# AnthonyDickson/HIVE

Hardware: AMD Instinct MI355X
Metric: frames/sec (depth+TSDF integrate) @640x480, 512^3 vol (higher is better)
Workload: dtype bf16; 1 GPU; synthetic 640x480x150 RGB (seeded room trajectory), host-resident uint8 frames uploaded in the timed region, DPT-Hybrid depth (seeded random weights: depth 1-7 m, bf16, hip engine) + 512x512x512 TSDF integrate, 107 frames/step; frames_total=4066, volume=512x512x512, tsdf_overlap=True, scaling_mode=weak

## Files before the change

### hive_amd/csrc/capi.hip

```cpp
#include <algorithm>

#include "hive_internal.hpp"

static thread_local std::string g_global_error;

void hive_set_global_error(const char *msg) { g_global_error = msg ? msg : ""; }

int hive_fail(hive_ctx *ctx, int code, const char *fmt, ...) {
    char buf[1024];
    va_list ap;
    va_start(ap, fmt);
    vsnprintf(buf, sizeof(buf), fmt, ap);
    va_end(ap);
    if (ctx)
        ctx->last_error = buf;
    else
        g_global_error = buf;
    return code;
}

int hive_reserve_device(hive_ctx *ctx, void **ptr, size_t *cur, size_t bytes) {
    if (*cur >= bytes && *ptr) return HIVE_OK;
    if (*ptr) {
        HIVE_CHECK_HIP(ctx, hipStreamSynchronize(ctx->stream));
// ... 103 lines not shown
            e = hipDeviceGetStreamPriorityRange(&least, &greatest);
            if (e == hipSuccess) e = hipStreamCreateWithPriority(&ctx->stream, hipStreamNonBlocking, least);
            ctx->owns_stream = true;
        } else {
            ctx->stream = (hipStream_t)stream;
        }
    }
    if (e == hipSuccess) e = hipMalloc((void **)&ctx->d_scalars, 4096 * sizeof(unsigned));
    if (e == hipSuccess) e = hipMemset(ctx->d_scalars, 0, 4096 * sizeof(unsigned));
    if (e == hipSuccess) e = hipMalloc(&ctx->d_zeros, 256);
    if (e == hipSuccess) e = hipMemset(ctx->d_zeros, 0, 256);
    if (e != hipSuccess) {
        int rc = hive_fail(nullptr, HIVE_ERR_DEVICE, "hive_ctx_create: %s", hipGetErrorString(e));
        delete ctx;
        return rc;
    }
    *out = ctx;
    return HIVE_OK;
}

int hive_ctx_destroy(hive_ctx *ctx) {
    if (!ctx) return HIVE_OK;
    {
        HIVE_ENTER(ctx);
        (void)hipStreamSynchronize(ctx->stream);
    for (auto &s : ctx->slots) {
        if (s.pinned) (void)hipHostFree(s.pinned);
        if (s.done) (void)hipEventDestroy(s.done);
    }
    for (auto ev : ctx->ev_pool) (void)hipEventDestroy(ev);
    if (ctx->d_scratch) (void)hipFree(ctx->d_scratch);
    if (ctx->d_frame) (void)hipFree(ctx->d_frame);
    if (ctx->d_batch) (void)hipFree(ctx->d_batch);
    if (ctx->d_gram) (void)hipFree(ctx->d_gram);
    if (ctx->d_splitk) (void)hipFree(ctx->d_splitk);
    if (ctx->d_splitk_count) (void)hipFree(ctx->d_splitk_count);
    if (ctx->d_in) (void)hipFree(ctx->d_in);
    if (ctx->d_scalars) (void)hipFree(ctx->d_scalars);
    if (ctx->h_pinned_small) (void)hipHostFree(ctx->h_pinned_small);
        if (ctx->d_zeros) (void)hipFree(ctx->d_zeros);
        if (ctx->owns_stream) (void)hipStreamDestroy(ctx->stream);
    }
    delete ctx;
    return HIVE_OK;
}

int hive_ctx_release_stream(hive_ctx *ctx) {
    if (!ctx) return hive_fail(nullptr, HIVE_ERR_INVALID, "ctx is NULL");
    ctx->owns_stream = false;
    return HIVE_OK;
}

int hive_ctx_set_stream(hive_ctx *ctx, void *stream) {
    HIVE_ENTER(ctx);
    if (!ctx) return hive_fail(nullptr, HIVE_ERR_INVALID, "ctx is NULL");
    HIVE_REQUIRE(ctx, stream != HIVE_STREAM_OWN && stream != HIVE_STREAM_OWN_LOW, "hive_ctx_set_stream: pass a hipStream_t (NULL = the default stream)");
    hipStream_t next = (hipStream_t)stream;
    if (next == ctx->stream) return HIVE_OK;
    hipEvent_t ev;
    HIVE_CHECK_HIP(ctx, hipEventCreateWithFlags(&ev, hipEventDisableTiming));
    hipError_t e = hipEventRecord(ev, ctx->stream);
    if (e == hipSuccess) e = hipStreamWaitEvent(next, ev, 0);
    (void)hipEventDestroy(ev);
    HIVE_CHECK_HIP(ctx, e);
    if (ctx->owns_stream) {
        (void)hipStreamSynchronize(ctx->stream);
// ... 82 lines not shown
```

### hive_amd/csrc/hive_internal.hpp

```cpp
#pragma once
#include <hip/hip_runtime.h>

#include <cstdarg>
#include <cstdint>
#include <cstdio>
#include <cstring>
#include <string>
#include <vector>

#include "../../include/hive_mi355x.h"

#define HIVE_WAVE 64

struct hive_staging_slot {
    void *pinned = nullptr;
    size_t bytes = 0;
    hipEvent_t done = nullptr;
    bool in_flight = false;
};

struct hive_ctx {
    int device = 0;
    int num_cus = 256;
    hipStream_t stream = nullptr;
    bool owns_stream = false;
    int round_mode = HIVE_ROUND_HALF_EVEN;
    std::string last_error;

    static constexpr int kSlots = 4;
    hive_staging_slot slots[kSlots];
    int next_slot = 0;

    void *d_scratch = nullptr;
    size_t scratch_bytes = 0;
    void *d_frame = nullptr;
    size_t frame_bytes = 0;
    void *d_batch = nullptr;
    size_t batch_bytes = 0;
    void *d_in = nullptr;
    size_t in_bytes = 0;
    int tsdf_scalars = 0;
    int tsdf_multi_scalars = 0;
    unsigned *d_scalars = nullptr;
    void *h_pinned_small = nullptr;
    void *d_zeros = nullptr;
    void *d_splitk = nullptr;
    size_t splitk_bytes = 0;
    unsigned *d_splitk_count = nullptr;
    void *d_gram = nullptr;
    size_t gram_bytes = 0;

    bool deterministic = false;
    int64_t n_splitk_launches = 0, n_deep_ring_launches = 0;

    bool timing = false;
    std::vector<hipEvent_t> ev_pool;
    size_t ev_used = 0;
    hipEvent_t last_start = nullptr, last_stop = nullptr;
};

int hive_fail(hive_ctx *ctx, int code, const char *fmt, ...);

struct hive_device_guard {
    int prev = -1;
    bool switched = false;
    explicit hive_device_guard(const hive_ctx *ctx) {
        if (!ctx) return;
        if (hipGetDevice(&prev) == hipSuccess && prev != ctx->device) switched = hipSetDevice(ctx->device) == hipSuccess;
    }
    ~hive_device_guard() {
        if (switched) (void)hipSetDevice(prev);
    }
    hive_device_guard(const hive_device_guard &) = delete;
    hive_device_guard &operator=(const hive_device_guard &) = delete;
};
// ... 93 lines not shown
```

### hive_amd/csrc/tsdf.hip

```cpp
#include "hive_internal.hpp"

#include <algorithm>
#include <cmath>
#include <cstdlib>
#include <type_traits>

struct FrameParams {
    float R[9];
    float T[3];
    float fx, fy, cx, cy;
    float ox, oy, oz, vs, trunc, obs_w;
    int X, Y, Z, H, W;
    int x_off;
    const uint2 *frame;
    const unsigned *tile_max;
    int tile_shift, tiles_x, tiles_y;
    int row_far;
    int fast_colour;
    unsigned long long *n_updated;
};

template <bool VEC>
__global__ __launch_bounds__(256) void prep_frame_kernel(const float *__restrict__ depth, const uint8_t *__restrict__ color, int H, int W, int tile_shift,
                                                         int tiles_x, uint2 *__restrict__ out, unsigned *__restrict__ tile_max, int tile_stride,
// ... 564 lines not shown
                vol_store4(v2 + idx, c, nrow);
            } else {
                vol_store4(v0 + plane + idx, w, nrow);
                vol_store4(v0 + 2 * plane + idx, c, nrow);
                vol_store4(v0 + 3 * plane + idx, c3, nrow);
                vol_store4(v0 + 4 * plane + idx, c4, nrow);
            }
        }
    }
    if (COUNT) {
        __shared__ unsigned wave_cnt[4];
        for (int off = 32; off > 0; off >>= 1) n_upd += __shfl_xor((int)n_upd, off);
        if (lane == 0) wave_cnt[threadIdx.x >> 6] = n_upd;
        __syncthreads();
        if (threadIdx.x == 0) {
            const unsigned total = wave_cnt[0] + wave_cnt[1] + wave_cnt[2] + wave_cnt[3];
            if (total) atomicAdd(p.n_updated + (size_t)(blockIdx.x % COUNT_SLOTS) * COUNT_STRIDE, (unsigned long long)total);
        }
    }
}

#ifndef HIVE_TSDF_MAXF
#define HIVE_TSDF_MAXF 4
#endif
constexpr int MAXF = HIVE_TSDF_MAXF;
static_assert(MAXF <= 4, "WorkItem::zz holds a 4-bit frame mask");
struct MultiParams {
    FrameParams f[MAXF];
    int nf;
    int frame_skip;
    int xcd_split;
    int bins_x;
    unsigned *clear_next;
    int lanes_along_x;
    int quad_interleave;
};

constexpr int MS_BASE = 2304, MS_STRIDE = 512, MS_NITEMS = MAXF, MS_HIST = 8, MS_CURSOR = MS_HIST + NBINS, MS_CLEAR = MS_CURSOR + NBINS;

__global__ __launch_bounds__(1024) void build_worklist_multi_kernel(MultiParams mp, WorkItem *__restrict__ items, unsigned *n_items, unsigned *hist) {
    __shared__ unsigned wave_sum[16];
    __shared__ unsigned block_base;
    __shared__ float dil[MAXF][MAX_TILES];
    __shared__ unsigned gmax[MAXF];
    __shared__ float gsum[MAXF];
    __shared__ unsigned bin_count[NBINS];
    constexpr int CHUNK = SEG_LANES * VPT;
    const FrameParams &p = mp.f[0];
    if (threadIdx.x < MAXF) gmax[threadIdx.x] = 0u, gsum[threadIdx.x] = 0.f;
    if (threadIdx.x < NBINS) bin_count[threadIdx.x] = 0u;
    __syncthreads();
    for (int f = 0; f < mp.nf; ++f) load_dilated_tiles(mp.f[f].tile_max, p.tiles_x, p.tiles_y, dil[f], &gmax[f], &gsum[f], threadIdx.x, 1024);
    __syncthreads();
    const long long row = (long long)blockIdx.x * 1024 + threadIdx.x;
    unsigned n_chunks = 0;
    int zstart = 0, z1 = 0, x = 0, y = 0;
    int fz0[MAXF], fz1[MAXF];
    float ax0 = 0.f, ay0 = 0.f, az0 = 0.f;
    auto frames_of = [&](int zs) {
        unsigned mask = 0;
#pragma unroll
        for (int f = 0; f < MAXF; ++f) mask |= (fz1[f] > zs && fz0[f] < zs + CHUNK) ? (1u << f) : 0u;
        return mask;
    };
    if (row < (long long)p.X * p.Y) {
        if (mp.lanes_along_x) {
            y = (int)(row / p.X);
            x = (int)(row % p.X);
        } else {
            x = (int)(row / p.Y);
            y = (int)(row % p.Y);
        }
        int lo = p.Z, hi = 0;
#pragma unroll
        for (int f = 0; f < MAXF; ++f) {
            fz0[f] = fz1[f] = 0;
            if (f < mp.nf) {
                const FrameParams &q = mp.f[f];
                const float tx = (q.ox + (float)(x + q.x_off) * q.vs) - q.T[0];
                const float ty = (q.oy + (float)y * q.vs) - q.T[1];
                const float ax = q.R[0] * tx + q.R[3] * ty;
                const float ay = q.R[1] * tx + q.R[4] * ty;
                const float az = q.R[2] * tx + q.R[5] * ty;
                if (f == 0) ax0 = ax, ay0 = ay, az0 = az;
                const bool row_far = p.row_far == 2 || (p.row_far == 1 && row_far_pays(gsum[f], gmax[f], p.tiles_x * p.tiles_y));
                const RowClip clip = clip_row(q, ax, ay, az, __uint_as_float(gmax[f]), row_far ? dil[f] : nullptr);
                if (clip.z1 > clip.z0) {
                    fz0[f] = clip.z0, fz1[f] = clip.z1;
                    lo = min(lo, clip.z0);
                    hi = max(hi, clip.z1);
                }
            }
        }
        if (hi > lo) {
            zstart = (lo / VPT) * VPT;
            z1 = hi;
            for (int zs = zstart; zs < z1; zs += CHUNK) n_chunks += frames_of(zs) ? 1u : 0u;
        }
    }
    const unsigned first = worklist_slots(n_chunks, n_items, wave_sum, &block_base);
    const int lane = threadIdx.x & 63;
    const unsigned quad_first = (unsigned)__shfl((int)first, lane & ~3);
    unsigned nq[4];
#pragma unroll
    for (int j = 0; j < 4; ++j) nq[j] = (unsigned)__shfl((int)n_chunks, (lane & ~3) + j);
    unsigned e = 0;
    if (n_chunks)
        for (int zs = zstart; zs < z1; zs += CHUNK) {
            const unsigned mask = frames_of(zs);
            if (!mask) continue;
            unsigned slot = quad_first;
            if (mp.quad_interleave) {
#pragma unroll
                for (int j = 0; j < 4; ++j) slot += min(nq[j], e) + ((j < (lane & 3) && nq[j] > e) ? 1u : 0u);
            } else {
                slot = first + e;
            }
            ++e;
            const float tz = (p.oz + (float)(zs + CHUNK / 2) * p.vs) - p.T[2];
            const float cz = az0 + p.R[8] * tz;
            const float v = cz > 1.0e-6f ? p.fy * ((ay0 + p.R[7] * tz) / cz) + p.cy : 0.f;
            const int bins_y = NBINS / mp.bins_x;
            int bin = min(max((int)(v * ((float)bins_y / (float)p.H)), 0), bins_y - 1);
            if (mp.bins_x > 1) {
                const float u = cz > 1.0e-6f ? p.fx * ((ax0 + p.R[6] * tz) / cz) + p.cx : 0.f;
                bin = bin * mp.bins_x + min(max((int)(u * ((float)mp.bins_x / (float)p.W)), 0), mp.bins_x - 1);
            }
            atomicAdd(&bin_count[bin], 1u);
            WorkItem it;
            it.xy = (unsigned)x | ((unsigned)y << 16);
            it.zz = (unsigned)zs | ((unsigned)(min(z1 - zs, CHUNK) - 1) << ITEM_NLIVE_SHIFT) | (mask << ITEM_MASK_SHIFT) | ((unsigned)bin << ITEM_BIN_SHIFT);
            items[slot] = it;
        }
    __syncthreads();
    if (threadIdx.x < NBINS && bin_count[threadIdx.x]) atomicAdd(hist + threadIdx.x, bin_count[threadIdx.x]);
}

__global__ __launch_bounds__(1024) void sort_worklist_kernel(const WorkItem *__restrict__ tmp, WorkItem *__restrict__ out, const unsigned *__restrict__ n_items_ptr,
                                                             const unsigned *__restrict__ hist, unsigned *cursor) {
    __shared__ unsigned base[NBINS], cnt[NBINS], gofs[NBINS];
    const unsigned n = *n_items_ptr;
    const unsigned i0 = blockIdx.x * 1024u;
    if (i0 >= n) return;
    if (threadIdx.x < NBINS) cnt[threadIdx.x] = 0u;
    if (threadIdx.x == 0) {
        unsigned a = 0;
        for (int b = 0; b < NBINS; ++b) {
            base[b] = a;
            a += hist[b];
        }
    }
    __syncthreads();
    const unsigned i = i0 + threadIdx.x;
    const int lane = threadIdx.x & 63;
    WorkItem it;
    it.xy = it.zz = 0u;
    unsigned bin = 0xffffffffu;
    if (i < n) {
        it = tmp[i];
        bin = it.zz >> ITEM_BIN_SHIFT;
    }
    unsigned rank = 0, wave_base = 0;
    unsigned long long todo = __ballot(i < n);
    while (todo) {
        const int leader = __ffsll((long long)todo) - 1;
        const unsigned b = (unsigned)__shfl((int)bin, leader);
        const unsigned long long m = __ballot(bin == b);
        unsigned wb = 0;
        if (lane == leader) wb = atomicAdd(&cnt[b], (unsigned)__popcll(m));
        wb = (unsigned)__shfl((int)wb, leader);
        if (bin == b) {
            rank = (unsigned)__popcll(m & ((1ull << lane) - 1ull));
            wave_base = wb;
        }
        todo &= ~m;
    }
    __syncthreads();
    if (threadIdx.x < NBINS && cnt[threadIdx.x]) gofs[threadIdx.x] = atomicAdd(cursor + threadIdx.x, cnt[threadIdx.x]);
    __syncthreads();
    if (i < n) out[base[bin] + gofs[bin] + wave_base + rank] = it;
}

#ifdef HIVE_TSDF_WAVES
#define HIVE_TSDF_OCC __attribute__((amdgpu_waves_per_eu(HIVE_TSDF_WAVES, HIVE_TSDF_WAVES)))
#else
#define HIVE_TSDF_OCC
#endif
template <int RM, int UPD>
__global__ __launch_bounds__(256) HIVE_TSDF_OCC void integrate_multi_kernel(MultiParams mp, const WorkItem *__restrict__ items, const unsigned *__restrict__ n_items_ptr,
                                                              float *__restrict__ v0, float *__restrict__ v1, float *__restrict__ v2) {
    constexpr int PER_WAVE = 64 / SEG_LANES, SEG_VOX = SEG_LANES * 4;
    typedef ItemShape Sh;
    typedef Sh::V V;
    __shared__ uint2 xchg[4 * PER_WAVE * SEG_VOX];
    const int lane = threadIdx.x & 63;
    const int seg = lane / SEG_LANES, sl = lane % SEG_LANES;
    const unsigned n_items = *n_items_ptr;
    const unsigned n_trips = (n_items + PER_WAVE - 1) / PER_WAVE;
    const unsigned per_xcd = mp.xcd_split ? (n_trips + 7u) / 8u : n_trips;
    const unsigned xcd = mp.xcd_split ? (blockIdx.x & 7u) : 0u;
    const unsigned local_block = mp.xcd_split ? (blockIdx.x >> 3) : blockIdx.x;
    const unsigned stride = (mp.xcd_split ? (gridDim.x >> 3) : gridDim.x) * 4;
    const unsigned trip_end = min(n_trips, (xcd + 1u) * per_xcd);
    const FrameParams &p0 = mp.f[0];
    const float trunc_rcp = refined_rcp(p0.trunc);
    if (blockIdx.x == 0 && (int)threadIdx.x < MS_CLEAR) mp.clear_next[threadIdx.x] = 0u;
    for (unsigned trip = xcd * per_xcd + local_block * 4 + (threadIdx.x >> 6); trip < trip_end; trip += stride) {
        const unsigned ii = trip * PER_WAVE + (unsigned)seg;
        WorkItem item;
        item.xy = item.zz = 0u;
        if (ii < n_items) item = items[ii];
        const int x = (int)(item.xy & 0xffffu), y = (int)(item.xy >> 16);
        const int zseg = (int)(item.zz & 0xffffu);
        const int zb = zseg + sl * VPT;
        const bool live = sl * VPT < item_nlive(item.zz);
        const int nrow = p0.Z - zb;
        const long long idx = ((long long)x * p0.Y + y) * p0.Z + zb;
        unsigned wave_frames = (item.zz >> ITEM_MASK_SHIFT) & 15u;
#pragma unroll
        for (int o = SEG_LANES; o < 64; o <<= 1) wave_frames |= (unsigned)__shfl_xor((int)wave_frames, o);
        wave_frames = mp.frame_skip ? (unsigned)__builtin_amdgcn_readfirstlane((int)wave_frames) : 0xffu;
        float t[VPT], w[VPT], cr[VPT], cg[VPT], cb[VPT];
        bool loaded = false;
        uint2 *mine = xchg + ((threadIdx.x >> 6) * PER_WAVE + seg) * SEG_VOX;
#pragma unroll 1
        for (int f = 0; f < mp.nf; ++f) {
            if (!((wave_frames >> f) & 1u)) continue;
            const FrameParams &p = mp.f[f];
            const float tx = (p.ox + (float)(x + p.x_off) * p.vs) - p.T[0];
            const float ty = (p.oy + (float)y * p.vs) - p.T[1];
            const float ax = p.R[0] * tx + p.R[3] * ty;
            const float ay = p.R[1] * tx + p.R[4] * ty;
            const float az = p.R[2] * tx + p.R[5] * ty;
            uint2 tex[4];
#pragma unroll
            for (int g = 0; g < 2; ++g) {
                V cz;
                int pix[Sh::NV];
                voxel_pixels<RM, V, Sh::NV, SEG_LANES>(p, ax, ay, az, zseg + sl + 2 * SEG_LANES * g, cz, pix);
// ... 216 lines not shown
    p.fy = K[4];
    p.cx = K[2];
    p.cy = K[5];
    p.ox = v->origin[0];
    p.oy = v->origin[1];
    p.oz = v->origin[2];
    p.vs = v->voxel_size;
    p.trunc = v->trunc;
    p.obs_w = obs_weight;
    p.X = (int)v->dim[0];
    p.x_off = (int)v->x_off;
    p.Y = (int)v->dim[1];
    p.Z = (int)v->dim[2];
    p.H = H;
    p.W = W;
    const TileGrid tg = tile_grid(H, W);
    p.tile_shift = tg.shift;
    p.tiles_x = tg.tiles_x;
    p.tiles_y = tg.tiles_y;
    {
        const char *e = getenv("HIVE_TSDF_ROW_FAR");
        p.row_far = e ? std::min(2, std::max(0, atoi(e))) : 1;
    }
    p.frame = nullptr;
    p.tile_max = nullptr;
    p.fast_colour = (v->round_mode == HIVE_ROUND_HALF_AWAY && obs_weight == 1.0f && v->unit_weights && env_flag("HIVE_TSDF_FAST_COLOUR", true)) ? 1 : 0;
    p.n_updated = nullptr;
}

struct PreparedFrames {
    const uint2 *texels;
    const unsigned *tile_max;
    int tile_stride;
};
static int prepare_batch(hive_tsdf *v, int n, const uint8_t *color, const float *depth, int H, int W, PreparedFrames *out) {
    hive_ctx *ctx = v->ctx;
    const size_t npx = (size_t)H * W;
    const TileGrid tg = tile_grid(H, W);
    const size_t tex_bytes = ((size_t)n * npx * sizeof(uint2) + 255) & ~(size_t)255;
    int rc = hive_reserve_device(ctx, &ctx->d_batch, &ctx->batch_bytes, tex_bytes + (size_t)n * MAX_TILES * sizeof(unsigned));
    if (rc) return rc;
    unsigned *d_tiles = (unsigned *)((char *)ctx->d_batch + tex_bytes);
    const bool vec = W % 4 == 0 && (uintptr_t)depth % 16 == 0 && (uintptr_t)color % 4 == 0;
    const dim3 grid((unsigned)(tg.tiles_x * tg.tiles_y), (unsigned)n);
    if (vec)
        hipLaunchKernelGGL(prep_frame_kernel<true>, grid, dim3(256), 0, ctx->stream, depth, color, H, W, tg.shift, tg.tiles_x, (uint2 *)ctx->d_batch, d_tiles, MAX_TILES,
                           (unsigned *)nullptr, 0);
    else
        hipLaunchKernelGGL(prep_frame_kernel<false>, grid, dim3(256), 0, ctx->stream, depth, color, H, W, tg.shift, tg.tiles_x, (uint2 *)ctx->d_batch, d_tiles, MAX_TILES,
                           (unsigned *)nullptr, 0);
    HIVE_CHECK_HIP(ctx, hipGetLastError());
    out->texels = (const uint2 *)ctx->d_batch;
    out->tile_max = d_tiles;
    out->tile_stride = MAX_TILES;
    return HIVE_OK;
}

static int launch_integrate_multi(hive_tsdf *v, int nf, int H, int W, const float K[9], const double *poses, float obs_weight, const PreparedFrames &prepared) {
    hive_ctx *ctx = v->ctx;
    const size_t npx = (size_t)H * W;
    int rc = HIVE_OK;
    static_assert(MS_CLEAR <= 256 && MS_CLEAR <= MS_STRIDE, "integrate_multi_kernel clears the next block with one workgroup of 256 threads");
    ctx->tsdf_multi_scalars ^= 1;
    unsigned *sc = ctx->d_scalars + MS_BASE + (ctx->tsdf_multi_scalars ? MS_STRIDE : 0);
    unsigned *idle_block = ctx->d_scalars + MS_BASE + (ctx->tsdf_multi_scalars ? 0 : MS_STRIDE);
    const uint2 *texels = prepared.texels;
    const unsigned *tiles = prepared.tile_max;
    const int tile_stride = prepared.tile_stride;
    const bool sorted = env_flag("HIVE_TSDF_SORT", true);
    MultiParams mp;
    mp.nf = nf;
    mp.frame_skip = env_flag("HIVE_TSDF_FRAME_SKIP", true) ? 1 : 0;
    mp.xcd_split = sorted ? 1 : 0;
    mp.clear_next = idle_block;
    const double *pose0 = poses;
    const bool auto_x = fabs(pose0[0 * 4 + 1]) <= fabs(pose0[1 * 4 + 1]);
    const char *lanes_env = getenv("HIVE_TSDF_LANES");
    mp.lanes_along_x = lanes_env ? (lanes_env[0] == 'x') : (auto_x ? 1 : 0);
    mp.quad_interleave = env_flag("HIVE_TSDF_QUAD", true) ? 1 : 0;
    {
        const char *e = getenv("HIVE_TSDF_BINS_X");
        int bx = e ? atoi(e) : 1;
        if (bx != 1 && bx != 2 && bx != 4 && bx != 8 && bx != 16) bx = 1;
        mp.bins_x = bx;
    }
    for (int f = 0; f < nf; ++f) {
        fill_frame_params(v, H, W, K, poses + 16 * (size_t)f, obs_weight, mp.f[f]);
        mp.f[f].frame = texels + (size_t)f * npx;
        mp.f[f].tile_max = tiles + (size_t)f * tile_stride;
#ifdef HIVE_TSDF_TUNING
        if (env_flag("HIVE_TSDF_TIMING_SAME_TEXELS", false)) mp.f[f].frame = texels;
#endif
    }
    for (int f = nf; f < MAXF; ++f) mp.f[f] = mp.f[0];
    const FrameParams &p = mp.f[0];
    const long long rows = (long long)p.X * p.Y;
    const long long seg = SEG_LANES * 4;
    const size_t max_items = (size_t)rows * (size_t)((p.Z + seg - 1) / seg);
    if ((rc = hive_reserve_device(ctx, &ctx->d_scratch, &ctx->scratch_bytes, 2 * max_items * sizeof(WorkItem)))) return rc;
    WorkItem *built = (WorkItem *)ctx->d_scratch, *items = sorted ? built + max_items : built;
    unsigned *n_items = sc + MS_NITEMS;
    v->last_n_items = n_items;
    hipLaunchKernelGGL(build_worklist_multi_kernel, dim3((unsigned)((rows + 1023) / 1024)), dim3(1024), 0, ctx->stream, mp, built, n_items, sc + MS_HIST);
    if (sorted)
        hipLaunchKernelGGL(sort_worklist_kernel, dim3((unsigned)((max_items + 1023) / 1024)), dim3(1024), 0, ctx->stream, (const WorkItem *)built, items,
                           (const unsigned *)n_items, (const unsigned *)(sc + MS_HIST), sc + MS_CURSOR);
    const long long max_trips = (long long)((max_items + 64 / SEG_LANES - 1) / (64 / SEG_LANES));
    const long long blocks = std::min<long long>((long long)ctx->num_cus * 8 * HIVE_GRID_MULT, (max_trips + 3) / 4);
    const dim3 grid((unsigned)((blocks + 7) / 8 * 8)), block(256);
    if ((rc = hive_time_begin(ctx))) return rc;
    const int upd = p.fast_colour ? 2 : (obs_weight == 1.0f ? 1 : 0);
#define HIVE_LAUNCH(RM, UPD) \
    hipLaunchKernelGGL((integrate_multi_kernel<RM, UPD>), grid, block, 0, ctx->stream, mp, (const WorkItem *)items, (const unsigned *)n_items, v->d_tsdf, v->d_weight, v->d_color)
    switch ((v->round_mode ? 3 : 0) + upd) {
        case 0: HIVE_LAUNCH(0, 0); break;
        case 1: HIVE_LAUNCH(0, 1); break;
        case 3: HIVE_LAUNCH(1, 0); break;
        case 4: HIVE_LAUNCH(1, 1); break;
        case 5: HIVE_LAUNCH(1, 2); break;
        default: return hive_fail(ctx, HIVE_ERR_STATE, "integrate: no kernel for round mode %d / update form %d", v->round_mode, upd);
    }
#undef HIVE_LAUNCH
    HIVE_CHECK_HIP(ctx, hipGetLastError());
    ++v->launches_seen;
    return hive_time_end(ctx);
}

template <bool ACCUM>
static int launch_integrate(hive_tsdf *v, float *accum, int H, int W, const float K[9], const double pose[16],
                            float obs_weight, bool count) {
    hive_ctx *ctx = v->ctx;
    FrameParams p;
    fill_frame_params(v, H, W, K, pose, obs_weight, p);
    p.frame = (const uint2 *)ctx->d_frame;
    p.tile_max = (const unsigned *)((const char *)ctx->d_frame + (((size_t)H * W * sizeof(uint2) + 255) & ~(size_t)255));
    p.n_updated = (unsigned long long *)(ctx->d_scalars + 128);
    if (count) HIVE_CHECK_HIP(ctx, hipMemsetAsync(p.n_updated, 0, COUNT_SLOTS * COUNT_STRIDE * sizeof(unsigned long long), ctx->stream));
    const long long rows = (long long)p.X * p.Y;
    float *a0 = ACCUM ? accum : v->d_tsdf;
    const long long seg = SEG_LANES * VPT;
    const size_t max_items = (size_t)rows * (size_t)((p.Z + seg - 1) / seg);
    int rc = hive_reserve_device(ctx, &ctx->d_scratch, &ctx->scratch_bytes, max_items * sizeof(WorkItem));
    if (rc) return rc;
    WorkItem *items = (WorkItem *)ctx->d_scratch;
    unsigned *n_items = tsdf_scalars(ctx) + 4;
    v->last_n_items = n_items;
// ... 204 lines not shown
        unsigned long long slots[COUNT_SLOTS * COUNT_STRIDE];
        HIVE_CHECK_HIP(ctx, hipMemcpyAsync(slots, ctx->d_scalars + 128, sizeof(slots), hipMemcpyDeviceToHost, ctx->stream));
        HIVE_CHECK_HIP(ctx, hipStreamSynchronize(ctx->stream));
        unsigned long long n = 0;
        for (int i = 0; i < COUNT_SLOTS; ++i) n += slots[i * COUNT_STRIDE];
        *n_updated = n;
    }
    return HIVE_OK;
}

int hive_tsdf_integrate_batch(hive_tsdf *vol, int n, const uint8_t *color, const float *depth, int H, int W,
                              const float K[9], const double *cam_poses, float obs_weight, int mem) {
    HIVE_ENTER(vol ? vol->ctx : nullptr);
    int rc = check_frame_args(vol, color, depth, H, W, K, cam_poses, mem);
    if (rc) return rc;
    HIVE_REQUIRE(vol->ctx, n >= 0, "integrate_batch: n must be >= 0");
    note_observations(vol, obs_weight, n);
    const size_t npx = (size_t)H * W;
    static const char *frames_env = getenv("HIVE_TSDF_FRAMES_PER_LAUNCH");
    const int group = frames_env ? std::max(1, std::min(MAXF, atoi(frames_env))) : MAXF;
    const bool multi = mem == HIVE_MEM_DEVICE && group > 1;
    const double max_side = voxel_extent(vol);
    static const char *cos_env = getenv("HIVE_TSDF_FUSE_COS");
    const double fuse_cos = cos_env ? atof(cos_env) : 0.809017;
    static const char *dist_env = getenv("HIVE_TSDF_FUSE_DIST");
    const double fuse_dist = dist_env ? atof(dist_env) : 0.25;
    auto fusable = [&](int a, int b) {
        const double *pa = cam_poses + 16 * (size_t)a, *pb = cam_poses + 16 * (size_t)b;
        const double dot = pa[2] * pb[2] + pa[6] * pb[6] + pa[10] * pb[10];
        const double na = sqrt(pa[2] * pa[2] + pa[6] * pa[6] + pa[10] * pa[10]), nb = sqrt(pb[2] * pb[2] + pb[6] * pb[6] + pb[10] * pb[10]);
        const double dx = pa[3] - pb[3], dy = pa[7] - pb[7], dz = pa[11] - pb[11];
        return dot >= fuse_cos * na * nb && dx * dx + dy * dy + dz * dz <= fuse_dist * fuse_dist * max_side * max_side;
    };
    vol->last_groups.clear();
    constexpr int PREP_CHUNK = 128;
    PreparedFrames chunk{nullptr, nullptr, 0};
    int prep_lo = 0, prep_hi = 0;
    int f = 0;
    while (f < n) {
        int nf = 1;
        if (multi)
            while (nf < group && f + nf < n && fusable(f, f + nf)) ++nf;
        if (nf > 1) {
            if (f + nf > prep_hi) {
                prep_lo = f;
                prep_hi = std::min(n, f + PREP_CHUNK);
                if ((rc = prepare_batch(vol, prep_hi - prep_lo, color + (size_t)prep_lo * npx * 3, depth + (size_t)prep_lo * npx, H, W, &chunk))) return rc;
            }
            PreparedFrames mine = chunk;
            mine.texels += (size_t)(f - prep_lo) * npx;
            mine.tile_max += (size_t)(f - prep_lo) * chunk.tile_stride;
            if ((rc = launch_integrate_multi(vol, nf, H, W, K, cam_poses + 16 * (size_t)f, obs_weight, mine))) return rc;
        } else {
            const uint8_t *d_color;
            const float *d_depth;
            if ((rc = prepare_frame(vol, color + f * npx * 3, depth + f * npx, H, W, mem, &d_color, &d_depth))) return rc;
            if ((rc = launch_integrate<false>(vol, nullptr, H, W, K, cam_poses + 16 * (size_t)f, obs_weight, false))) return rc;
        }
        vol->last_groups.push_back(nf);
        f += nf;
    }
    vol->n_verts = vol->n_faces = -1;
    return HIVE_OK;
}

int hive_tsdf_last_batch_groups(hive_tsdf *vol, int *sizes, int capacity, int *n_groups) {
    if (!vol) return hive_fail(nullptr, HIVE_ERR_INVALID, "vol is NULL");
    HIVE_REQUIRE(vol->ctx, n_groups && capacity >= 0 && (sizes || capacity == 0), "last_batch_groups: bad arguments");
    *n_groups = (int)vol->last_groups.size();
    for (int i = 0; i < capacity && i < *n_groups; ++i) sizes[i] = vol->last_groups[i];
    return HIVE_OK;
}

int hive_tsdf_last_sweep_items(hive_tsdf *vol, uint64_t *n_items, int *segment_voxels) {
    HIVE_ENTER(vol ? vol->ctx : nullptr);
    if (!vol) return hive_fail(nullptr, HIVE_ERR_INVALID, "vol is NULL");
    hive_ctx *ctx = vol->ctx;
    HIVE_REQUIRE(ctx, n_items, "last_sweep_items: NULL argument");
    HIVE_REQUIRE(ctx, vol->last_n_items, "last_sweep_items: no sweep has run on this volume");
    unsigned n = 0;
    HIVE_CHECK_HIP(ctx, hipMemcpyAsync(&n, vol->last_n_items, sizeof(n), hipMemcpyDeviceToHost, ctx->stream));
    HIVE_CHECK_HIP(ctx, hipStreamSynchronize(ctx->stream));
    *n_items = n;
    if (segment_voxels) *segment_voxels = SEG_LANES * VPT;
    return HIVE_OK;
}

int hive_tsdf_get_volume(hive_tsdf *v, float *h_tsdf, float *h_color, float *h_weight) {
    HIVE_ENTER(v ? v->ctx : nullptr);
    if (!v) return hive_fail(nullptr, HIVE_ERR_INVALID, "vol is NULL");
    hive_ctx *ctx = v->ctx;
    const size_t bytes = (size_t)v->n * sizeof(float);
    if (h_tsdf) HIVE_CHECK_HIP(ctx, hipMemcpyAsync(h_tsdf, v->d_tsdf, bytes, hipMemcpyDefault, ctx->stream));
// ... 108 lines not shown
```

Before: 1377 frames/s.

## Batch worklist build and sort across many fused sweeps per launch

Instead of building and sorting a worklist per fused frame group right before each integrate launch, the batch path now plans all groups up front and builds and sorts worklists for up to 64 sweeps in one 2D-grid launch each. Tile dilation is precomputed once per frame in a new kernel, so the build kernel only loads dilated tiles when row clipping uses them. The aim is fewer small launches and better GPU fill for the build and sort phases. In exchange it needs much larger list memory (capped by an env var, default 1 GiB), a double-buffered scalar-block scheme with multi-block clearing, and MultiParams uploaded to the device.

```diff
diff --git a/hive_amd/csrc/capi.hip b/hive_amd/csrc/capi.hip
--- a/hive_amd/csrc/capi.hip
+++ b/hive_amd/csrc/capi.hip
@@ -159,6 +159,8 @@
     if (ctx->d_scratch) (void)hipFree(ctx->d_scratch);
     if (ctx->d_frame) (void)hipFree(ctx->d_frame);
     if (ctx->d_batch) (void)hipFree(ctx->d_batch);
+    if (ctx->d_lists) (void)hipFree(ctx->d_lists);
+    if (ctx->d_sweep_blocks) (void)hipFree(ctx->d_sweep_blocks);
     if (ctx->d_gram) (void)hipFree(ctx->d_gram);
     if (ctx->d_splitk) (void)hipFree(ctx->d_splitk);
     if (ctx->d_splitk_count) (void)hipFree(ctx->d_splitk_count);
diff --git a/hive_amd/csrc/hive_internal.hpp b/hive_amd/csrc/hive_internal.hpp
--- a/hive_amd/csrc/hive_internal.hpp
+++ b/hive_amd/csrc/hive_internal.hpp
@@ -40,7 +40,11 @@
     void *d_in = nullptr;
     size_t in_bytes = 0;
     int tsdf_scalars = 0;
-    int tsdf_multi_scalars = 0;
+    void *d_lists = nullptr;
+    size_t lists_bytes = 0;
+    unsigned *d_sweep_blocks = nullptr;
+    int sweep_set = 0;
+    int sweep_dirty[2] = {0, 0};
     unsigned *d_scalars = nullptr;
     void *h_pinned_small = nullptr;
     void *d_zeros = nullptr;
diff --git a/hive_amd/csrc/tsdf.hip b/hive_amd/csrc/tsdf.hip
--- a/hive_amd/csrc/tsdf.hip
+++ b/hive_amd/csrc/tsdf.hip
@@ -620,13 +620,32 @@
     int xcd_split;
     int bins_x;
     unsigned *clear_next;
+    int clear_blocks;
     int lanes_along_x;
     int quad_interleave;
+    const unsigned *dil[MAXF];
 };
 
-constexpr int MS_BASE = 2304, MS_STRIDE = 512, MS_NITEMS = MAXF, MS_HIST = 8, MS_CURSOR = MS_HIST + NBINS, MS_CLEAR = MS_CURSOR + NBINS;
-
-__global__ __launch_bounds__(1024) void build_worklist_multi_kernel(MultiParams mp, WorkItem *__restrict__ items, unsigned *n_items, unsigned *hist) {
+constexpr int MS_STRIDE = 512, MS_NITEMS = MAXF, MS_HIST = 8, MS_CURSOR = MS_HIST + NBINS, MS_CLEAR = MS_CURSOR + NBINS;
+constexpr int MAX_CHUNK_SWEEPS = 64;
+static_assert(MS_CLEAR <= MS_STRIDE, "a scalar block holds the work-list length, the band histogram and the sort cursors");
+
+constexpr int DIL_STRIDE = MAX_TILES + 4;
+__global__ __launch_bounds__(1024) void dilate_tiles_kernel(const unsigned *__restrict__ tile_max, int tile_stride, int tiles_x, int tiles_y, unsigned *__restrict__ out) {
+    __shared__ float dil[MAX_TILES];
+    __shared__ unsigned gmax;
+    __shared__ float gsum;
+    if (threadIdx.x == 0) gmax = 0u, gsum = 0.f;
+    __syncthreads();
+    load_dilated_tiles(tile_max + (size_t)blockIdx.x * tile_stride, tiles_x, tiles_y, dil, &gmax, &gsum, threadIdx.x, 1024);
+    __syncthreads();
+    unsigned *o = out + (size_t)blockIdx.x * DIL_STRIDE;
+    for (int t = threadIdx.x; t < tiles_x * tiles_y; t += 1024) o[t] = __float_as_uint(dil[t]);
+    if (threadIdx.x == 0) o[MAX_TILES] = gmax, o[MAX_TILES + 1] = __float_as_uint(gsum);
+}
+
+__global__ __launch_bounds__(1024) void build_worklist_multi_kernel(const MultiParams *__restrict__ mps, WorkItem *__restrict__ lists, size_t list_items,
+                                                                    unsigned *__restrict__ blocks) {
     __shared__ unsigned wave_sum[16];
     __shared__ unsigned block_base;
     __shared__ float dil[MAXF][MAX_TILES];
@@ -634,11 +653,22 @@
     __shared__ float gsum[MAXF];
     __shared__ unsigned bin_count[NBINS];
     constexpr int CHUNK = SEG_LANES * VPT;
+    const MultiParams &mp = mps[blockIdx.y];
+    WorkItem *items = lists + 2 * list_items * blockIdx.y;
+    unsigned *n_items = blocks + (size_t)blockIdx.y * MS_STRIDE + MS_NITEMS, *hist = blocks + (size_t)blockIdx.y * MS_STRIDE + MS_HIST;
     const FrameParams &p = mp.f[0];
-    if (threadIdx.x < MAXF) gmax[threadIdx.x] = 0u, gsum[threadIdx.x] = 0.f;
+    if ((int)threadIdx.x < mp.nf) {
+        const unsigned *rec = mp.dil[threadIdx.x];
+        gmax[threadIdx.x] = rec[MAX_TILES];
+        gsum[threadIdx.x] = __uint_as_float(rec[MAX_TILES + 1]);
+    }
     if (threadIdx.x < NBINS) bin_count[threadIdx.x] = 0u;
     __syncthreads();
-    for (int f = 0; f < mp.nf; ++f) load_dilated_tiles(mp.f[f].tile_max, p.tiles_x, p.tiles_y, dil[f], &gmax[f], &gsum[f], threadIdx.x, 1024);
+    const int tiles = p.tiles_x * p.tiles_y;
+    auto row_far_of = [&](int f) { return p.row_far == 2 || (p.row_far == 1 && row_far_pays(gsum[f], gmax[f], tiles)); };
+    for (int f = 0; f < mp.nf; ++f)
+        if (row_far_of(f))
+            for (int t = threadIdx.x; t < tiles; t += 1024) dil[f][t] = __uint_as_float(mp.dil[f][t]);
     __syncthreads();
     const long long row = (long long)blockIdx.x * 1024 + threadIdx.x;
     unsigned n_chunks = 0;
@@ -671,8 +701,7 @@
                 const float ay = q.R[1] * tx + q.R[4] * ty;
                 const float az = q.R[2] * tx + q.R[5] * ty;
                 if (f == 0) ax0 = ax, ay0 = ay, az0 = az;
-                const bool row_far = p.row_far == 2 || (p.row_far == 1 && row_far_pays(gsum[f], gmax[f], p.tiles_x * p.tiles_y));
-                const RowClip clip = clip_row(q, ax, ay, az, __uint_as_float(gmax[f]), row_far ? dil[f] : nullptr);
+                const RowClip clip = clip_row(q, ax, ay, az, __uint_as_float(gmax[f]), row_far_of(f) ? dil[f] : nullptr);
                 if (clip.z1 > clip.z0) {
                     fz0[f] = clip.z0, fz1[f] = clip.z1;
                     lo = min(lo, clip.z0);
@@ -724,13 +753,15 @@
     if (threadIdx.x < NBINS && bin_count[threadIdx.x]) atomicAdd(hist + threadIdx.x, bin_count[threadIdx.x]);
 }
 
-__global__ __launch_bounds__(1024) void sort_worklist_kernel(const WorkItem *__restrict__ tmp, WorkItem *__restrict__ out, const unsigned *__restrict__ n_items_ptr,
-                                                             const unsigned *__restrict__ hist, unsigned *cursor) {
+__global__ __launch_bounds__(1024) void sort_worklist_kernel(WorkItem *__restrict__ lists, size_t list_items, unsigned *__restrict__ blocks) {
     __shared__ unsigned base[NBINS], cnt[NBINS], gofs[NBINS];
-    const unsigned n = *n_items_ptr;
-    const unsigned i0 = blockIdx.x * 1024u;
-    if (i0 >= n) return;
-    if (threadIdx.x < NBINS) cnt[threadIdx.x] = 0u;
+    const WorkItem *tmp = lists + 2 * list_items * blockIdx.y;
+    WorkItem *out = lists + 2 * list_items * blockIdx.y + list_items;
+    unsigned *sc = blocks + (size_t)blockIdx.y * MS_STRIDE;
+    const unsigned *hist = sc + MS_HIST;
+    unsigned *cursor = sc + MS_CURSOR;
+    const unsigned n = sc[MS_NITEMS];
+    if (blockIdx.x * 1024u >= n) return;
     if (threadIdx.x == 0) {
         unsigned a = 0;
         for (int b = 0; b < NBINS; ++b) {
@@ -738,35 +769,38 @@
             a += hist[b];
         }
     }
-    __syncthreads();
-    const unsigned i = i0 + threadIdx.x;
     const int lane = threadIdx.x & 63;
-    WorkItem it;
-    it.xy = it.zz = 0u;
-    unsigned bin = 0xffffffffu;
-    if (i < n) {
-        it = tmp[i];
-        bin = it.zz >> ITEM_BIN_SHIFT;
-    }
-    unsigned rank = 0, wave_base = 0;
-    unsigned long long todo = __ballot(i < n);
-    while (todo) {
-        const int leader = __ffsll((long long)todo) - 1;
-        const unsigned b = (unsigned)__shfl((int)bin, leader);
-        const unsigned long long m = __ballot(bin == b);
-        unsigned wb = 0;
-        if (lane == leader) wb = atomicAdd(&cnt[b], (unsigned)__popcll(m));
-        wb = (unsigned)__shfl((int)wb, leader);
-        if (bin == b) {
-            rank = (unsigned)__popcll(m & ((1ull << lane) - 1ull));
-            wave_base = wb;
-        }
-        todo &= ~m;
-    }
-    __syncthreads();
-    if (threadIdx.x < NBINS && cnt[threadIdx.x]) gofs[threadIdx.x] = atomicAdd(cursor + threadIdx.x, cnt[threadIdx.x]);
-    __syncthreads();
-    if (i < n) out[base[bin] + gofs[bin] + wave_base + rank] = it;
+    for (unsigned i0 = blockIdx.x * 1024u; i0 < n; i0 += gridDim.x * 1024u) {
+        if (threadIdx.x < NBINS) cnt[threadIdx.x] = 0u;
+        __syncthreads();
+        const unsigned i = i0 + threadIdx.x;
+        WorkItem it;
+        it.xy = it.zz = 0u;
+        unsigned bin = 0xffffffffu;
+        if (i < n) {
+            it = tmp[i];
+            bin = it.zz >> ITEM_BIN_SHIFT;
+        }
+        unsigned rank = 0, wave_base = 0;
+        unsigned long long todo = __ballot(i < n);
+        while (todo) {
+            const int leader = __ffsll((long long)todo) - 1;
+            const unsigned b = (unsigned)__shfl((int)bin, leader);
+            const unsigned long long m = __ballot(bin == b);
+            unsigned wb = 0;
+            if (lane == leader) wb = atomicAdd(&cnt[b], (unsigned)__popcll(m));
+            wb = (unsigned)__shfl((int)wb, leader);
+            if (bin == b) {
+                rank = (unsigned)__popcll(m & ((1ull << lane) - 1ull));
+                wave_base = wb;
+            }
+            todo &= ~m;
+        }
+        __syncthreads();
+        if (threadIdx.x < NBINS && cnt[threadIdx.x]) gofs[threadIdx.x] = atomicAdd(cursor + threadIdx.x, cnt[threadIdx.x]);
+        __syncthreads();
+        if (i < n) out[base[bin] + gofs[bin] + wave_base + rank] = it;
+    }
 }
 
 #ifdef HIVE_TSDF_WAVES
@@ -792,7 +826,8 @@
     const unsigned trip_end = min(n_trips, (xcd + 1u) * per_xcd);
     const FrameParams &p0 = mp.f[0];
     const float trunc_rcp = refined_rcp(p0.trunc);
-    if (blockIdx.x == 0 && (int)threadIdx.x < MS_CLEAR) mp.clear_next[threadIdx.x] = 0u;
+    if (blockIdx.x == 0)
+        for (int i = threadIdx.x; i < mp.clear_blocks * MS_CLEAR; i += 256) mp.clear_next[(i / MS_CLEAR) * MS_STRIDE + i % MS_CLEAR] = 0u;
     for (unsigned trip = xcd * per_xcd + local_block * 4 + (threadIdx.x >> 6); trip < trip_end; trip += stride) {
         const unsigned ii = trip * PER_WAVE + (unsigned)seg;
         WorkItem item;
@@ -1075,15 +1110,18 @@
     const uint2 *texels;
     const unsigned *tile_max;
     int tile_stride;
+    const unsigned *dilated;
 };
 static int prepare_batch(hive_tsdf *v, int n, const uint8_t *color, const float *depth, int H, int W, PreparedFrames *out) {
     hive_ctx *ctx = v->ctx;
     const size_t npx = (size_t)H * W;
     const TileGrid tg = tile_grid(H, W);
     const size_t tex_bytes = ((size_t)n * npx * sizeof(uint2) + 255) & ~(size_t)255;
-    int rc = hive_reserve_device(ctx, &ctx->d_batch, &ctx->batch_bytes, tex_bytes + (size_t)n * MAX_TILES * sizeof(unsigned));
+    const size_t tile_bytes = (size_t)n * MAX_TILES * sizeof(unsigned);
+    int rc = hive_reserve_device(ctx, &ctx->d_batch, &ctx->batch_bytes, tex_bytes + tile_bytes + (size_t)n * DIL_STRIDE * sizeof(unsigned));
     if (rc) return rc;
     unsigned *d_tiles = (unsigned *)((char *)ctx->d_batch + tex_bytes);
+    unsigned *d_dilated = (unsigned *)((char *)ctx->d_batch + tex_bytes + tile_bytes);
     const bool vec = W % 4 == 0 && (uintptr_t)depth % 16 == 0 && (uintptr_t)color % 4 == 0;
     const dim3 grid((unsigned)(tg.tiles_x * tg.tiles_y), (unsigned)n);
     if (vec)
@@ -1092,69 +1130,117 @@
     else
         hipLaunchKernelGGL(prep_frame_kernel<false>, grid, dim3(256), 0, ctx->stream, depth, color, H, W, tg.shift, tg.tiles_x, (uint2 *)ctx->d_batch, d_tiles, MAX_TILES,
                            (unsigned *)nullptr, 0);
+    hipLaunchKernelGGL(dilate_tiles_kernel, dim3((unsigned)n), dim3(1024), 0, ctx->stream, (const unsigned *)d_tiles, MAX_TILES, tg.tiles_x, tg.tiles_y, d_dilated);
     HIVE_CHECK_HIP(ctx, hipGetLastError());
     out->texels = (const uint2 *)ctx->d_batch;
     out->tile_max = d_tiles;
     out->tile_stride = MAX_TILES;
-    return HIVE_OK;
-}
-
-static int launch_integrate_multi(hive_tsdf *v, int nf, int H, int W, const float K[9], const double *poses, float obs_weight, const PreparedFrames &prepared) {
+    out->dilated = d_dilated;
+    return HIVE_OK;
+}
+
+struct SweepChunk {
+    std::vector<MultiParams> mp;
+    WorkItem *lists = nullptr;
+    size_t list_items = 0;
+    unsigned *blocks = nullptr;
+    bool sorted = true;
+    int launched = 0;
+};
+
+static size_t sweep_list_items(const hive_tsdf *v) {
+    const size_t seg = SEG_LANES * VPT;
+    return (size_t)v->dim[0] * (size_t)v->dim[1] * (((size_t)v->dim[2] + seg - 1) / seg);
+}
+
+static int build_sweep_lists(hive_tsdf *v, const std::vector<int> &frames, const std::vector<int> &nfs, int H, int W, const float K[9], const double *poses,
+                             float obs_weight, const PreparedFrames &prepared, SweepChunk &ch) {
     hive_ctx *ctx = v->ctx;
     const size_t npx = (size_t)H * W;
+    const int ns = (int)frames.size();
     int rc = HIVE_OK;
-    static_assert(MS_CLEAR <= 256 && MS_CLEAR <= MS_STRIDE, "integrate_multi_kernel clears the next block with one workgroup of 256 threads");
-    ctx->tsdf_multi_scalars ^= 1;
-    unsigned *sc = ctx->d_scalars + MS_BASE + (ctx->tsdf_multi_scalars ? MS_STRIDE : 0);
-    unsigned *idle_block = ctx->d_scalars + MS_BASE + (ctx->tsdf_multi_scalars ? 0 : MS_STRIDE);
-    const uint2 *texels = prepared.texels;
-    const unsigned *tiles = prepared.tile_max;
-    const int tile_stride = prepared.tile_stride;
-    const bool sorted = env_flag("HIVE_TSDF_SORT", true);
-    MultiParams mp;
-    mp.nf = nf;
-    mp.frame_skip = env_flag("HIVE_TSDF_FRAME_SKIP", true) ? 1 : 0;
-    mp.xcd_split = sorted ? 1 : 0;
-    mp.clear_next = idle_block;
-    const double *pose0 = poses;
-    const bool auto_x = fabs(pose0[0 * 4 + 1]) <= fabs(pose0[1 * 4 + 1]);
+    if (ns < 1 || ns > MAX_CHUNK_SWEEPS) return hive_fail(ctx, HIVE_ERR_STATE, "integrate_batch: a chunk of %d sweeps", ns);
+    constexpr size_t set_words = (size_t)MAX_CHUNK_SWEEPS * MS_STRIDE;
+    if (!ctx->d_sweep_blocks) {
+        HIVE_CHECK_HIP(ctx, hipMalloc((void **)&ctx->d_sweep_blocks, 2 * set_words * sizeof(unsigned) + MAX_CHUNK_SWEEPS * sizeof(MultiParams)));
+        HIVE_CHECK_HIP(ctx, hipMemsetAsync(ctx->d_sweep_blocks, 0, 2 * set_words * sizeof(unsigned), ctx->stream));
+        ctx->sweep_set = 0;
+        ctx->sweep_dirty[0] = ctx->sweep_dirty[1] = 0;
+    }
+    MultiParams *d_mp = (MultiParams *)(ctx->d_sweep_blocks + 2 * set_words);
+    ctx->sweep_set ^= 1;
+    const int mine = ctx->sweep_set, other = mine ^ 1;
+    ch.blocks = ctx->d_sweep_blocks + (size_t)mine * set_words;
+    ch.sorted = env_flag("HIVE_TSDF_SORT", true);
+    ch.launched = 0;
+    ch.list_items = sweep_list_items(v);
+    ch.mp.assign((size_t)ns, MultiParams());
     const char *lanes_env = getenv("HIVE_TSDF_LANES");
-    mp.lanes_along_x = lanes_env ? (lanes_env[0] == 'x') : (auto_x ? 1 : 0);
-    mp.quad_interleave = env_flag("HIVE_TSDF_QUAD", true) ? 1 : 0;
+    int bins_x = 1;
     {
         const char *e = getenv("HIVE_TSDF_BINS_X");
-        int bx = e ? atoi(e) : 1;
-        if (bx != 1 && bx != 2 && bx != 4 && bx != 8 && bx != 16) bx = 1;
-        mp.bins_x = bx;
-    }
-    for (int f = 0; f < nf; ++f) {
-        fill_frame_params(v, H, W, K, poses + 16 * (size_t)f, obs_weight, mp.f[f]);
-        mp.f[f].frame = texels + (size_t)f * npx;
-        mp.f[f].tile_max = tiles + (size_t)f * tile_stride;
+        const int bx = e ? atoi(e) : 1;
+        if (bx == 2 || bx == 4 || bx == 8 || bx == 16) bins_x = bx;
+    }
+    for (int s = 0; s < ns; ++s) {
+        MultiParams &mp = ch.mp[(size_t)s];
+        const int nf = nfs[(size_t)s], f0 = frames[(size_t)s];
+        mp.nf = nf;
+        mp.frame_skip = env_flag("HIVE_TSDF_FRAME_SKIP", true) ? 1 : 0;
+        mp.xcd_split = ch.sorted ? 1 : 0;
+        mp.bins_x = bins_x;
+        mp.clear_next = ctx->d_sweep_blocks + (size_t)other * set_words;
+        mp.clear_blocks = s == ns - 1 ? ctx->sweep_dirty[other] : 0;
+        const double *pose0 = poses + 16 * (size_t)f0;
+        const bool auto_x = fabs(pose0[0 * 4 + 1]) <= fabs(pose0[1 * 4 + 1]);
+        mp.lanes_along_x = lanes_env ? (lanes_env[0] == 'x') : (auto_x ? 1 : 0);
+        mp.quad_interleave = env_flag("HIVE_TSDF_QUAD", true) ? 1 : 0;
+        for (int f = 0; f < nf; ++f) {
+            fill_frame_params(v, H, W, K, pose0 + 16 * (size_t)f, obs_weight, mp.f[f]);
+            mp.f[f].frame = prepared.texels + (size_t)(f0 + f) * npx;
+            mp.f[f].tile_max = prepared.tile_max + (size_t)(f0 + f) * prepared.tile_stride;
+            mp.dil[f] = prepared.dilated + (size_t)(f0 + f) * DIL_STRIDE;
 #ifdef HIVE_TSDF_TUNING
-        if (env_flag("HIVE_TSDF_TIMING_SAME_TEXELS", false)) mp.f[f].frame = texels;
+            if (env_flag("HIVE_TSDF_TIMING_SAME_TEXELS", false)) mp.f[f].frame = mp.f[0].frame;
 #endif
-    }
-    for (int f = nf; f < MAXF; ++f) mp.f[f] = mp.f[0];
+        }
+        for (int f = nf; f < MAXF; ++f) mp.f[f] = mp.f[0], mp.dil[f] = mp.dil[0];
+    }
+    ctx->sweep_dirty[mine] = ns;
+    ctx->sweep_dirty[other] = 0;
+    if ((rc = hive_reserve_device(ctx, &ctx->d_lists, &ctx->lists_bytes, 2 * (size_t)ns * ch.list_items * sizeof(WorkItem)))) return rc;
+    ch.lists = (WorkItem *)ctx->d_lists;
+    if ((rc = hive_upload(ctx, d_mp, ch.mp.data(), (size_t)ns * sizeof(MultiParams)))) return rc;
+    const long long rows = (long long)v->dim[0] * v->dim[1];
+    hipLaunchKernelGGL(build_worklist_multi_kernel, dim3((unsigned)((rows + 1023) / 1024), (unsigned)ns), dim3(1024), 0, ctx->stream, (const MultiParams *)d_mp, ch.lists,
+                       ch.list_items, ch.blocks);
+    if (ch.sorted) {
+        const long long tiles = (long long)((ch.list_items + 1023) / 1024);
+        const long long wgs = std::max<long long>(1, std::min<long long>((tiles + 7) / 8, ((long long)ctx->num_cus * 8 + ns - 1) / ns));
+        hipLaunchKernelGGL(sort_worklist_kernel, dim3((unsigned)wgs, (unsigned)ns), dim3(1024), 0, ctx->stream, ch.lists, ch.list_items, ch.blocks);
+    }
+    HIVE_CHECK_HIP(ctx, hipGetLastError());
+    return HIVE_OK;
+}
+
+static int launch_integrate_sweep(hive_tsdf *v, SweepChunk &ch, float obs_weight) {
+    hive_ctx *ctx = v->ctx;
+    int rc = HIVE_OK;
+    if (ch.launched >= (int)ch.mp.size()) return hive_fail(ctx, HIVE_ERR_STATE, "integrate_batch: no list was built for this sweep");
+    const size_t s = (size_t)ch.launched++;
+    const MultiParams &mp = ch.mp[s];
     const FrameParams &p = mp.f[0];
-    const long long rows = (long long)p.X * p.Y;
-    const long long seg = SEG_LANES * 4;
-    const size_t max_items = (size_t)rows * (size_t)((p.Z + seg - 1) / seg);
-    if ((rc = hive_reserve_device(ctx, &ctx->d_scratch, &ctx->scratch_bytes, 2 * max_items * sizeof(WorkItem)))) return rc;
-    WorkItem *built = (WorkItem *)ctx->d_scratch, *items = sorted ? built + max_items : built;
-    unsigned *n_items = sc + MS_NITEMS;
+    const size_t max_items = ch.list_items;
+    const WorkItem *items = ch.lists + 2 * s * max_items + (ch.sorted ? max_items : 0);
+    const unsigned *n_items = ch.blocks + s * MS_STRIDE + MS_NITEMS;
     v->last_n_items = n_items;
-    hipLaunchKernelGGL(build_worklist_multi_kernel, dim3((unsigned)((rows + 1023) / 1024)), dim3(1024), 0, ctx->stream, mp, built, n_items, sc + MS_HIST);
-    if (sorted)
-        hipLaunchKernelGGL(sort_worklist_kernel, dim3((unsigned)((max_items + 1023) / 1024)), dim3(1024), 0, ctx->stream, (const WorkItem *)built, items,
-                           (const unsigned *)n_items, (const unsigned *)(sc + MS_HIST), sc + MS_CURSOR);
     const long long max_trips = (long long)((max_items + 64 / SEG_LANES - 1) / (64 / SEG_LANES));
     const long long blocks = std::min<long long>((long long)ctx->num_cus * 8 * HIVE_GRID_MULT, (max_trips + 3) / 4);
     const dim3 grid((unsigned)((blocks + 7) / 8 * 8)), block(256);
     if ((rc = hive_time_begin(ctx))) return rc;
     const int upd = p.fast_colour ? 2 : (obs_weight == 1.0f ? 1 : 0);
 #define HIVE_LAUNCH(RM, UPD) \
-    hipLaunchKernelGGL((integrate_multi_kernel<RM, UPD>), grid, block, 0, ctx->stream, mp, (const WorkItem *)items, (const unsigned *)n_items, v->d_tsdf, v->d_weight, v->d_color)
+    hipLaunchKernelGGL((integrate_multi_kernel<RM, UPD>), grid, block, 0, ctx->stream, mp, items, n_items, v->d_tsdf, v->d_weight, v->d_color)
     switch ((v->round_mode ? 3 : 0) + upd) {
         case 0: HIVE_LAUNCH(0, 0); break;
         case 1: HIVE_LAUNCH(0, 1); break;
@@ -1425,33 +1511,57 @@
         const double dx = pa[3] - pb[3], dy = pa[7] - pb[7], dz = pa[11] - pb[11];
         return dot >= fuse_cos * na * nb && dx * dx + dy * dy + dz * dz <= fuse_dist * fuse_dist * max_side * max_side;
     };
+    struct Group {
+        int f, nf;
+    };
+    std::vector<Group> plan;
     vol->last_groups.clear();
-    constexpr int PREP_CHUNK = 128;
-    PreparedFrames chunk{nullptr, nullptr, 0};
-    int prep_lo = 0, prep_hi = 0;
-    int f = 0;
-    while (f < n) {
+    for (int f = 0; f < n;) {
         int nf = 1;
         if (multi)
             while (nf < group && f + nf < n && fusable(f, f + nf)) ++nf;
+        plan.push_back(Group{f, nf});
+        vol->last_groups.push_back(nf);
+        f += nf;
+    }
+    size_t list_cap = (size_t)1 << 30;
+    if (const char *e = getenv("HIVE_TSDF_LIST_BYTES")) list_cap = (size_t)strtoull(e, nullptr, 10);
+    const size_t per_sweep = 2 * sweep_list_items(vol) * sizeof(WorkItem);
+    const int chunk_sweeps = env_flag("HIVE_TSDF_BATCH_LISTS", true) ? (int)std::max<size_t>(1, std::min<size_t>(MAX_CHUNK_SWEEPS, list_cap / per_sweep)) : 1;
+    constexpr int PREP_CHUNK = 128;
+    PreparedFrames prepared{nullptr, nullptr, 0, nullptr};
+    int prep_lo = 0, prep_hi = 0;
+    SweepChunk lists;
+    size_t lists_end = 0;
+    std::vector<int> sweep_frames, sweep_nfs;
+    for (size_t g = 0; g < plan.size(); ++g) {
+        const int f = plan[g].f, nf = plan[g].nf;
         if (nf > 1) {
             if (f + nf > prep_hi) {
                 prep_lo = f;
                 prep_hi = std::min(n, f + PREP_CHUNK);
-                if ((rc = prepare_batch(vol, prep_hi - prep_lo, color + (size_t)prep_lo * npx * 3, depth + (size_t)prep_lo * npx, H, W, &chunk))) return rc;
+                if ((rc = prepare_batch(vol, prep_hi - prep_lo, color + (size_t)prep_lo * npx * 3, depth + (size_t)prep_lo * npx, H, W, &prepared))) return rc;
             }
-            PreparedFrames mine = chunk;
-            mine.texels += (size_t)(f - prep_lo) * npx;
-            mine.tile_max += (size_t)(f - prep_lo) * chunk.tile_stride;
-            if ((rc = launch_integrate_multi(vol, nf, H, W, K, cam_poses + 16 * (size_t)f, obs_weight, mine))) return rc;
+            if (g >= lists_end) {
+                sweep_frames.clear();
+                sweep_nfs.clear();
+                size_t e = g;
+                for (; e < plan.size() && (int)sweep_frames.size() < chunk_sweeps; ++e) {
+                    if (plan[e].nf == 1) continue;
+                    if (plan[e].f + plan[e].nf > prep_hi) break;
+                    sweep_frames.push_back(plan[e].f - prep_lo);
+                    sweep_nfs.push_back(plan[e].nf);
+                }
+                lists_end = e;
+                if ((rc = build_sweep_lists(vol, sweep_frames, sweep_nfs, H, W, K, cam_poses + 16 * (size_t)prep_lo, obs_weight, prepared, lists))) return rc;
+            }
+            if ((rc = launch_integrate_sweep(vol, lists, obs_weight))) return rc;
         } else {
             const uint8_t *d_color;
             const float *d_depth;
             if ((rc = prepare_frame(vol, color + f * npx * 3, depth + f * npx, H, W, mem, &d_color, &d_depth))) return rc;
             if ((rc = launch_integrate<false>(vol, nullptr, H, W, K, cam_poses + 16 * (size_t)f, obs_weight, false))) return rc;
         }
-        vol->last_groups.push_back(nf);
-        f += nf;
     }
     vol->n_verts = vol->n_faces = -1;
     return HIVE_OK;
```

Measured after the change: 1381 frames/s (median of 6 runs). Within noise of the previous version (+0.3%).
